# Shunpoco/mini-kube-scheduler

Measured on AMD Instinct MI355X. Metric: pod×node filter+score evals/sec and pods scheduled/sec at 100k nodes, 1/2/4/8 GPU, higher is better.
Workload: dtype u32; 1 GPU; C: 100000 nodes x 100000 pods (100000 per GPU, strong scaling), NU+NN, batched, every pair evaluated, node-sharded over 1 GPU; nodes=100000, pods=100000, pods_per_gpu=100000, plugins=NU+NN, parallelism=node-shard1

## Files before the change

mini-kube-scheduler_amd/csrc/ms_capi.cpp:

```cpp
#include <hip/hip_runtime.h>

#include <algorithm>
#include <cstdio>
#include <cstdlib>
#include <cstring>
#include <functional>
#include <mutex>
#include <new>
#include <string>
#include <type_traits>
#include <unordered_map>
#include <vector>

#include "ms_ctx.h"
#include "ms_nam_layout.h"

using namespace msgpu;

ms_ctx::~ms_ctx() {
    (void)hipSetDevice(cfg.device);
    comm_free(this);
    if (stream) (void)hipStreamSynchronize(stream);
    if (copy_stream) (void)hipStreamSynchronize(copy_stream);
}
// ... 40 lines not shown
    if (fenced) ++c->fence_seq;
    std::unordered_map<uint32_t, uint32_t> last;
    last.reserve(batch.size() * 2);
    for (uint32_t i = 0; i < batch.size(); ++i) last[batch[i].local] = i;
    std::vector<NodeDelta> uniq;
    uniq.reserve(last.size());
    for (uint32_t i = 0; i < batch.size(); ++i)
        if (last[batch[i].local] == i) uniq.push_back(batch[i]);
    int rc = ensure_delta_cap(c, (uint32_t)uniq.size());
    if (rc) return rc;
    MS_HIP(c, hipStreamSynchronize(c->stream));
    std::memcpy(c->h_deltas, uniq.data(), sizeof(NodeDelta) * uniq.size());
    MS_HIP(c, hipMemcpyAsync(c->d_deltas, c->h_deltas, sizeof(NodeDelta) * uniq.size(),
                             hipMemcpyHostToDevice, c->stream));
    MS_HIP(c, launch_apply_deltas(c->t, c->d_deltas, (uint32_t)uniq.size(), c->stream));
    MS_HIP(c, launch_build_planes(c->t, c->d_deltas, (uint32_t)uniq.size(), c->stream));
    ++c->ctx_seq;
    return MS_OK;
}

hipStream_t pick_stream(ms_ctx *c, void *s) { return s ? (hipStream_t)s : c->stream; }

int order_after_ctx_stream(ms_ctx *c, hipStream_t s) {
    const int fenced = comm_fence_reads(c, c->stream);
    if (fenced < 0) return fenced;
    if (fenced) ++c->fence_seq;
    if (s == c->stream) return MS_OK;
    if (s == c->ordered_stream && c->ordered_seq == c->ctx_seq && c->ordered_fence == c->fence_seq)
        return MS_OK;
    MS_HIP(c, made(c->ev_order.ensure()));
    hipError_t e = hipEventRecord(c->ev_order, c->stream);
// ... 246 lines not shown
        MS_HIP(c, launch_decode(d_pods + s0, nb, c->d_keys, nullptr, c->present_dev, d_res + s0, s));
        if (commit) MS_HIP(c, launch_apply_binds(c->t, d_pods + s0, nb, d_res + s0, s));
    }
    return MS_OK;
}

int sweep_locked(ms_ctx *c, uint32_t n_pods, const ms_pod_rec *d_pods, unsigned long long *keys, uint32_t *flags,
                 hipStream_t s, hipEvent_t done) {
    const uint32_t seed32 = seed32_of(c->cfg.seed);
    if (c->cfg.plugin_set == MS_PLUGINS_NU_TT_NN)
        return fail(c, MS_E_INVAL, "TaintToleration shards combine by summaries (ms_tt_summaries_device), not keys");
    if (c->cfg.plugin_set == MS_PLUGINS_NU_NN_NAM)
        return fail(c, MS_E_INVAL, "multi-term NodeAffinity shards exchange rescale tables first "
                                   "(ms_nam_segment_device, ms_nam_keys_device)");
    if (c->cfg.plugin_set == MS_PLUGINS_NU_NN) {
        MS_HIP(c, launch_sweep_pp(c->t, c->rows_dev, d_pods, n_pods, seed32, keys, nullptr, c->present_dev,
                                  c->num_cus, s, 0, done));
        return MS_OK;
    } else if (c->cfg.plugin_set == MS_PLUGINS_NU_NN_NA) {
        MS_HIP(c, launch_fill_keys(keys, n_pods, c->present_dev ? kKeyListed : 0ull, s));
        MS_HIP(c, hipMemsetAsync(flags, 0, sizeof(uint32_t) * n_pods, s));
        MS_HIP(c, launch_sweep_na(c->t, c->rows_dev, d_pods, n_pods, seed32, c->w_nn, c->w_na, keys, flags,
                                  c->num_cus, s));
    } else {
        MS_HIP(c, launch_fill_keys(keys, n_pods, c->present_dev ? kKeyListed : 0ull, s));
        if (flags) MS_HIP(c, hipMemsetAsync(flags, 0, sizeof(uint32_t) * n_pods, s));
        MS_HIP(c, launch_sweep_full(c->t, c->rows_dev, d_pods, n_pods, seed32, keys, flags, c->num_cus, s));
    }
    if (done) MS_HIP(c, hipEventRecord(done, s));
    return MS_OK;
}
// ... 10 lines not shown
    const uint32_t B = c->batch_cap;
    const bool fused = c->cfg.plugin_set == MS_PLUGINS_NU_NN;
    if (c->cfg.plugin_set == MS_PLUGINS_NU_NN_NAM) {
        int rc = nam_cycle_locked(c, n_pods, d_pods, d_res, commit, s);
        if (rc) return rc;
        if (done) MS_HIP(c, hipEventRecord(done, s));
        return MS_OK;
    }
    if (c->cfg.plugin_set == MS_PLUGINS_NU_TT_NN) {
        int rc = tt_cycle_locked(c, n_pods, d_pods, nullptr, d_res, commit, s);
        if (rc) return rc;
        if (done) MS_HIP(c, hipEventRecord(done, s));
        return MS_OK;
    }
    if (fused && c->rows_dev <= kPpMaxFusedRows) {
        MS_HIP(c, launch_sweep_pp(c->t, c->rows_dev, d_pods, n_pods, seed32_of(c->cfg.seed), nullptr, d_res,
                                  c->present_dev, c->num_cus, s, commit, done));
        return MS_OK;
    }
    const bool late_commit = commit && !plugins_stateless(c);
    for (uint32_t s0 = 0; s0 < n_pods; s0 += B) {
        const uint32_t nb = std::min(B, n_pods - s0);
        if (fused) {
            MS_HIP(c, launch_sweep_pp(c->t, c->rows_dev, d_pods + s0, nb, seed32_of(c->cfg.seed), c->d_keys,
                                      d_res + s0, c->present_dev, c->num_cus, s, commit));
            continue;
        }
        const bool want_flags = c->cfg.plugin_set != MS_PLUGINS_NU_NN;
        int rc = sweep_locked(c, nb, d_pods + s0, c->d_keys, want_flags ? c->d_flags : nullptr, s);
        if (rc) return rc;
        MS_HIP(c, decode_for(c, d_pods + s0, nb, c->d_keys, want_flags ? c->d_flags : nullptr, c->present_dev,
                             d_res + s0, s));
        if (commit && !late_commit) MS_HIP(c, launch_apply_binds(c->t, d_pods + s0, nb, d_res + s0, s));
    }
    if (late_commit) MS_HIP(c, launch_apply_binds(c->t, d_pods, n_pods, d_res, s));
    if (done) MS_HIP(c, hipEventRecord(done, s));
    return MS_OK;
}

// ... 108 lines not shown
            }
        });
    };
    ++c->ctx_seq;
    ck.count(MS_PH_CHUNKS, parts);
    for (uint32_t i = 0; i < parts; ++i) {
        ms_pod_compact *z = c->h_podz;
        par(beg(i), beg(i + 1), [&](uint32_t a, uint32_t b) {
            if constexpr (std::is_same<PodIn, ms_pod_compact>::value) {
                std::memcpy(z + a, pods + a, sizeof(ms_pod_compact) * (b - a));
            } else {
                for (uint32_t j = a; j < b; ++j) std::memcpy(&z[j], &pods[j], sizeof(ms_pod_compact));
            }
        });
        ck.lap(MS_PH_STAGE_IN);
        MS_HIP(c, launch_sweep_pp_compact(c->t, c->rows_dev, c->h_podz + beg(i), beg(i + 1) - beg(i),
                                          seed32_of(c->cfg.seed), c->h_resz + beg(i), c->present_dev, c->num_cus, s));
        MS_HIP(c, hipEventRecord(c->ev_cyc[i], s));
        ck.lap(MS_PH_LAUNCH);
        if (i > 0) {
            MS_HIP(c, hipEventSynchronize(c->ev_cyc[i - 1]));
            ck.lap(MS_PH_WAIT);
            move_out(i - 1);
            ck.lap(MS_PH_STAGE_OUT);
        }
    }
    MS_HIP(c, hipEventSynchronize(c->ev_cyc[parts - 1]));
    ck.lap(MS_PH_WAIT);
    move_out(parts - 1);
    ck.lap(MS_PH_STAGE_OUT);
    return MS_OK;
// ... 89 lines not shown
                     (void **)&t.nz_mem};
    const size_t bytes[] = {n + kColumnPad, n + kColumnPad, n + kColumnPad, n + kColumnPad, n * 4, n * 4, n * 4,
                            n * 8,          n * 8,          n * 8,          n * 8,          n * 8, n * 8};
    static_assert(sizeof(cols) / sizeof(cols[0]) == sizeof(bytes) / sizeof(bytes[0]), "one size per column");
    size_t off[sizeof(bytes) / sizeof(bytes[0])], total = 0;
    for (size_t i = 0; i < sizeof(bytes) / sizeof(bytes[0]); ++i) {
        off[i] = total;
        total += (bytes[i] + 255) & ~(size_t)255;
    }
    total = (total + (2u << 20) - 1) & ~(size_t)((2u << 20) - 1);
    bool ok = c->d_table.alloc(total);
    if (ok)
        for (size_t i = 0; i < sizeof(bytes) / sizeof(bytes[0]); ++i)
            *cols[i] = static_cast<char *>(c->d_table.get()) + off[i];
    t.gcap = (uint32_t)((n + kGroupRows - 1) / kGroupRows);
    ok = ok && c->d_planes.alloc((size_t)kPlanes * t.gcap);
    if (!ok) return bail(MS_E_OOM, "node table allocation");
    t.planes = c->d_planes;
    const size_t b = c->batch_cap;
    ok = ensure_stage(c, c->batch_cap) == MS_OK && c->d_keys.alloc(b) && c->d_flags.alloc(b) && c->d_one.alloc(1) &&
         c->d_overflow.alloc(kStatsBytes / sizeof(uint32_t));
    if (!ok) return bail(MS_E_OOM, "staging allocation");
    if (launch_init_table(t, c->stream) != hipSuccess || launch_build_planes(t, nullptr, 0, c->stream) != hipSuccess)
        return bail(MS_E_HIP, "table init launch");
    if (hipMemsetAsync(c->d_overflow, 0, kStatsBytes, c->stream) != hipSuccess) return bail(MS_E_HIP, "memset");
    if (hipStreamSynchronize(c->stream) != hipSuccess) return bail(MS_E_HIP, "table init");
    *out = c;
    return MS_OK;
}

int ms_destroy(ms_ctx *c) {
    if (!c) return MS_E_INVAL;
#ifdef MS_VSTAMPS
    {
        uint32_t st[64] = {};
        (void)hipSetDevice(c->cfg.device);
        (void)hipStreamSynchronize(c->stream);
        if (hipMemcpy(st, c->d_overflow, kStatsBytes, hipMemcpyDeviceToHost) == hipSuccess) {
// ... 680 lines not shown
```

mini-kube-scheduler_amd/csrc/ms_comm.cpp:

```cpp
#include <rccl/rccl.h>

#include <algorithm>
#include <chrono>
#include <cstdio>
#include <cstdlib>
#include <cstring>
#include <deque>
#include <new>

#include "ms_ctx.h"

#ifdef MS_COMM_LOOPBACK
#include "ms_comm_loopback.h"
#define CCL(fn) lb_##fn
#else
#define CCL(fn) fn
#endif

namespace msgpu {

namespace {

constexpr uint32_t kPipeMax = 8;
static_assert(kPipeMax <= kMaxSliceJobs, "a full drain is one slice-decode launch");
// ... 295 lines not shown
    uint32_t si = 0;
    hipStream_t X = nullptr;
    int rc = prepare_locked(c, n, s, si, X);
    if (rc) return rc;
    host_tick(m, 0, tp);
    if (co && (!m.stash.on || m.stash.X != X)) {
        rc = flush_stash(c);
        if (rc) return rc;
        m.stash = CommState::Stash{true, n, si, pods, results, X};
        return MS_OK;
    }
    ShardSlot &sl = m.slot[si];
    if (co) {
        const CommState::Stash st = m.stash;
        m.stash.on = false;
        MS_HIP(c, launch_sweep_pp2(c->t, c->rows_dev, st.pods, st.n, m.slot[st.si].keys, pods, n, sl.keys,
                                   seed32_of(c->cfg.seed), c->present_dev, c->num_cus, X, m.ev_swept[si]));
        host_tick(m, 1, tp);
        m.reads_outstanding = true;
        rc = collective_locked(c, st.si, m.ev_swept[si], st.n, st.pods, st.results, tp);
        if (rc) return rc;
        return collective_locked(c, si, nullptr, n, pods, results, tp);
    }
    const int ps = c->cfg.plugin_set;
    if (ps == MS_PLUGINS_NU_TT_NN) {
        rc = tt2_sharded_sweep(c, si, n, pods, X);
        if (rc == MS_OK && hipEventRecord(m.ev_swept[si], X) != hipSuccess) rc = fail(c, MS_E_HIP, "event record");
    } else {
        rc = sweep_locked(c, n, pods, sl.keys, ps == MS_PLUGINS_NU_NN ? nullptr : sl.flags, X, m.ev_swept[si]);
    }
    if (rc) return rc;
// ... 251 lines not shown
```

mini-kube-scheduler_amd/csrc/ms_ctx.h:

```cpp
#pragma once

#include <hip/hip_runtime.h>

#include <chrono>
#include <cstdint>
#include <memory>
#include <mutex>
#include <string>
#include <type_traits>
#include <vector>

#include "ms_copy_pool.h"
#include "ms_internal.h"
#include "ms_owned.h"

namespace msgpu {
struct CommState;

template <class T>
constexpr size_t kElemBytes = sizeof(std::conditional_t<std::is_void<T>::value, char, T>);

template <class T>
struct DevMem {
    using handle = T *;
// ... 46 lines not shown
using msgpu::DRow;
using msgpu::Event;
using msgpu::NodeDelta;
using msgpu::NodeTable;
using msgpu::PinnedBuf;
using msgpu::Stream;

struct ms_ctx {
    ms_config cfg{};
    Stream stream;
    Stream copy_stream;
    int num_cus = 0;
    NodeTable t{};
    DevBuf<void> d_table;
    DevBuf<uint32_t> d_planes;
    ~ms_ctx();

    std::unique_ptr<msgpu::CopyPool> copy_pool;

    std::mutex delta_mu;
    std::vector<NodeDelta> pending;
    std::vector<uint8_t> present;
    uint32_t present_count = 0;
    uint32_t rows_used = 0;
    uint32_t rows_dev = 0, present_dev = 0;

    std::mutex sched_mu;

    uint32_t batch_cap = 0, stage_cap = 0, compact_cap = 0;
    DevBuf<ms_pod_compact> d_podc;
// ... 117 lines not shown
```

mini-kube-scheduler_amd/csrc/ms_internal.h:

```cpp
#pragma once

#include <hip/hip_runtime.h>
#include <stdint.h>

#include "minisched_gpu.h"

namespace msgpu {

constexpr uint8_t kNodeUnschedulable = 0x01;
constexpr uint8_t kNodeAbsent = 0x80;

constexpr int kNunnThreads = 256;
constexpr int kNunnSlots = 16;
constexpr int kNunnTile = kNunnThreads * kNunnSlots;

constexpr int kFullThreads = 256;
constexpr int kFullSlots = 4;
constexpr int kFullWaveTile = 64 * kFullSlots;
constexpr int kFullTile = kFullThreads * kFullSlots;

constexpr uint32_t kGolden32 = 0x9E3779B1u;

constexpr uint32_t kColumnPad = 64;

// ... 38 lines not shown

constexpr uint32_t kGroupRows = 30;
enum : uint32_t {
    kPlaneD0 = 0,
    kPlaneD1,
    kPlaneD2,
    kPlaneD3,
    kPlaneSched,
    kPlanePresent,
    kPlaneOver,
    kPlaneDigitPres,
    kPlaneDigitSched,
    kPlanes
};

struct NodeDelta {
    uint32_t local;
    uint32_t absent;
    ms_node_rec rec;
};
static_assert(sizeof(ms_node_rec) == 64, "ms_node_rec layout");
static_assert(sizeof(ms_pod_rec) == 40, "ms_pod_rec layout");
static_assert(sizeof(ms_result) == 24, "ms_result layout");
static_assert(sizeof(ms_pod_compact) == 8, "ms_pod_compact layout");
static_assert(sizeof(ms_result_compact) == 8, "ms_result_compact layout");

constexpr unsigned long long kKeyListed = 1ull;

__host__ __device__ inline uint32_t fmix32(uint32_t h) {
    h ^= h >> 16;
// ... 36 lines not shown
};
struct NamLayout;
hipError_t launch_nam_segment(const NodeTable &t, uint32_t n_rows, const ms_pod_rec *pods, uint32_t n_pods,
                              const void *sets, uint32_t n_sets, const NamLayout &L, void *scratch, void *out,
                              hipStream_t s);
hipError_t launch_nam_identity(void *out, uint32_t n, hipStream_t s);
hipError_t launch_nam_compose(const void *in, uint32_t stride, uint32_t n, uint32_t n_pods, int32_t skip_to,
                              void *out, uint8_t *m_in, hipStream_t s);
hipError_t launch_nam_keys(const NodeTable &t, uint32_t n_rows, const ms_pod_rec *pods, uint32_t n_pods,
                           const void *sets, uint32_t n_sets, uint32_t seed32, uint32_t w_nn, uint32_t w_na,
                           const void *after, const uint8_t *m_in, uint32_t listed, const NamLayout &L,
                           void *scratch, unsigned long long *keys, hipStream_t s);

hipError_t launch_apply_deltas(const NodeTable &t, const NodeDelta *d_deltas, uint32_t n, hipStream_t s);
hipError_t launch_init_table(const NodeTable &t, hipStream_t s);
hipError_t launch_sweep_pp(const NodeTable &t, uint32_t n_rows, const ms_pod_rec *pods, uint32_t n_pods,
                           uint32_t seed32, unsigned long long *keys, ms_result *results, uint32_t present,
                           int num_cus, hipStream_t s, int commit = 0, hipEvent_t done = nullptr);
hipError_t launch_sweep_pp2(const NodeTable &t, uint32_t n_rows, const ms_pod_rec *pods1, uint32_t n1,
                            unsigned long long *keys1, const ms_pod_rec *pods2, uint32_t n2, unsigned long long *keys2,
                            uint32_t seed32, uint32_t present, int num_cus, hipStream_t s, hipEvent_t done);
hipError_t launch_sweep_pp_compact(const NodeTable &t, uint32_t n_rows, const ms_pod_compact *pods, uint32_t n_pods,
                                   uint32_t seed32, ms_result_compact *results, uint32_t present, int num_cus,
                                   hipStream_t s);
constexpr uint32_t kPpMaxFusedRows = 16u * 64u * 4u * kGroupRows;
hipError_t launch_build_planes(const NodeTable &t, const NodeDelta *d_deltas, uint32_t n, hipStream_t s);
hipError_t launch_fill_keys(unsigned long long *keys, uint32_t n, unsigned long long v, hipStream_t s);
hipError_t launch_sweep_na(const NodeTable &t, uint32_t n_rows, const ms_pod_rec *pods, uint32_t n_pods,
                           uint32_t seed32, uint32_t w_nn, uint32_t w_na, unsigned long long *keys, uint32_t *fkeys,
                           int num_cus, hipStream_t s);
hipError_t launch_decode_na(const ms_pod_rec *pods, uint32_t n_pods, const unsigned long long *keys,
                            const uint32_t *fkeys, uint32_t present_nodes, uint32_t seed32, uint32_t w_nn,
                            uint32_t w_na, ms_result *out, hipStream_t s, const uint32_t *present_dev = nullptr);
hipError_t launch_sweep_full(const NodeTable &t, uint32_t n_rows, const ms_pod_rec *pods, uint32_t n_pods,
                             uint32_t seed32, unsigned long long *keys, uint32_t *flags, int num_cus,
                             hipStream_t s);
hipError_t launch_build_drows(const NodeTable &t, uint32_t n_rows, uint32_t n_total, hipStream_t s);
hipError_t launch_decode(const ms_pod_rec *pods, uint32_t n_pods, const unsigned long long *keys,
                         const uint32_t *flags, uint32_t present_nodes, ms_result *out, hipStream_t s,
                         const uint32_t *present_dev = nullptr);

// ... 106 lines not shown
```

mini-kube-scheduler_amd/csrc/ms_sweep_pp.hip:

```cpp
#include <hip/hip_ext.h>

#include <algorithm>
#include <cstdlib>

#include "ms_device.h"

namespace msgpu {

namespace {

template <typename F>
constexpr uint32_t truth3(F f) {
    uint32_t t = 0;
    for (int i = 0; i < 8; ++i)
        if (f((i >> 2) & 1, (i >> 1) & 1, i & 1)) t |= 1u << i;
    return t;
}
constexpr uint32_t kXnorAnd = truth3([](int a, int b, int c) { return c && a == b; });
constexpr uint32_t kSelect = truth3([](int a, int b, int c) { return c ? a : b; });

constexpr uint32_t kTailShare = 4;

constexpr int kPpWords = 4;
constexpr int kPpWordsSmall = 8;
// ... 122 lines not shown
    if (__ballot(found) != 0) return (1ull << 32) | wave_max_u32_dpp(h);
    return 0;
}

__device__ __forceinline__ uint2 pod_entry(const ms_pod_rec *__restrict__ pods, uint32_t p, uint32_t seed32,
                                           uint32_t pstride, uint32_t base10) {
    const uint2 pr = *reinterpret_cast<const uint2 *>(reinterpret_cast<const char *>(pods) + (size_t)p * pstride);
    const int dig = (int)(int8_t)(pr.y & 0xFFu);
    const bool isd = (uint32_t)dig <= 9u;
    const uint32_t info = (isd ? (uint32_t)dig : 14u) | (((pr.y >> 8) & 0xFFu) ? 16u : 0u);
    const uint32_t p0 = isd ? ((uint32_t)dig + 10u - base10) % 10u : 30u;
    return make_uint2(tb_pod(seed32, pr.x), info | ((pr.y & 0xFFu) << 8) | (p0 << 16));
}

constexpr uint32_t kPpClasses = 20;
constexpr uint32_t kPpSortWords = 72;
constexpr uint32_t kPpSortMin = 80;

__device__ __forceinline__ uint32_t pod_class(uint32_t info) {
    const uint32_t p0 = (info >> 16) & 31u;
    return p0 < 10u ? p0 + ((info & 16u) ? 10u : 0u) : kPpClasses;
}

template <int KW, int NW>
__device__ __forceinline__ bool run_setup(const Word (&W)[KW], uint32_t info, uint32_t (&B)[NW * 3]) {
    const Pod qc = pod_bits(0u, info);
    uint32_t m[NW], fb = 0;
    bool has = false;
#pragma unroll
    for (int k = 0; k < NW; ++k) {
        m[k] = match10(W[k], qc);
// ... 79 lines not shown
            if (mine && u != 0u) atomicMax(&lds[pb + pi], (11ull << 32) | u);
            u64 redo = __ballot(mine && u == 0u);
            while (redo) {
                const uint32_t l = (uint32_t)__builtin_ctzll(redo);
                redo &= redo - 1ull;
                const uint32_t t = rev3(l >> 3);
                const Pod qs = pod_bits((uint32_t)__builtin_amdgcn_readlane((int)a_l, (int)(j + t)),
                                        (uint32_t)__builtin_amdgcn_readlane((int)info_l, (int)(j + t)));
                const u64 v = pod_slow<KW, NW, MODE == kModeFix>(W, Wt, TAIL && ((pb + j) >> 3) % tshare == tidx, qs);
                if (lane == 0 && v) atomicMax(&lds[pb + j + t], v);
            }
        }
    }
}

template <int KW, int NW, int MODE, bool TAIL>
__device__ __forceinline__ void sweep_range(const Word (&W)[KW], const Word &Wt, uint32_t tpt, uint32_t tshare,
                                            uint32_t tidx, const uint2 *pinfo, const uint32_t *rb, bool runs,
                                            uint32_t np, uint32_t lane, u64 *lds) {
    constexpr bool RUN = MODE != kModeGen && NW > 0 && KW == kPpWords;
    const bool cut = RUN && runs;
    for (uint32_t c = cut ? 0u : kPpClasses; c <= kPpClasses; ++c) {
        const uint32_t beg = cut ? (uint32_t)__builtin_amdgcn_readfirstlane((int)rb[c]) : 0u;
        const uint32_t end = cut ? (uint32_t)__builtin_amdgcn_readfirstlane((int)rb[c + 1]) : np;
        if (beg >= end) continue;
        uint32_t B[RUN ? NW * 3 : 1] = {};
        bool form = false;
        if constexpr (RUN)
            if (c < kPpClasses)
                form = run_setup<KW, NW>(W, (uint32_t)__builtin_amdgcn_readfirstlane((int)pinfo[beg].y), B);
        sweep_pods<KW, NW, MODE, TAIL>(W, Wt, tpt, tshare, tidx, pinfo, beg, end, form, B, lane, lds);
    }
}

__host__ __device__ inline uint32_t tail_pods(uint32_t ng, uint32_t waves) {
    if (ng == 0) return 0u;
    const uint32_t wlast = (ng + 63u) / 64u - 1u, tail_n = ng - wlast * 64u;
    const uint32_t tpt = tail_n <= 8u ? 8u : 0u;
    if (!tpt) return 0u;
    if (waves <= 4u) return tpt;
    const uint32_t wv_t = wlast % waves;
    const uint32_t tshare = kTailShare < waves - wv_t ? kTailShare : waves - wv_t;
    uint32_t L[4] = {0, 0, 0, 0};
    for (uint32_t w = 0; w < waves && w <= wlast; ++w) L[w & 3u] += 16u * ((wlast - w) / waves + 1u);
// ... 7 lines not shown
    for (uint32_t i = 0; i < tshare; ++i) L[(wv_t + i) & 3u] += eps;
    return mx() < m0 ? tpt : 0u;
}

struct PpJob2 {
    const ms_pod_rec *pods;
    u64 *keys;
    uint32_t n_pods, nblk1;
};

template <int KW, bool TP>
__global__ __launch_bounds__(64 * kPpMaxWaves) void k_sweep_nunn_pp(
    const uint32_t *__restrict__ planes, uint32_t gstride, uint32_t n_groups, uint32_t node_base,
    const ms_pod_rec *__restrict__ pods1, uint32_t n_pods1, uint32_t chunk, uint32_t seed32, u64 *__restrict__ keys1,
    int atomic_keys, ms_result *__restrict__ results, uint32_t present, NodeTable tab, int commit,
    uint32_t pstride, ms_result_compact *__restrict__ resc, PpJob2 j2, int fix_ok, uint32_t xtra) {
    extern __shared__ u64 lds[];
    uint2 *pinfo = reinterpret_cast<uint2 *>(lds + chunk + (xtra ? 8u : 0u));
    const uint32_t lane = lane_id();
    const uint32_t wv = (uint32_t)__builtin_amdgcn_readfirstlane((int)(threadIdx.x >> 6));
    const bool second = j2.pods && blockIdx.x >= j2.nblk1;
    const ms_pod_rec *__restrict__ pods = second ? j2.pods : pods1;
    const uint32_t n_pods = second ? j2.n_pods : n_pods1;
    u64 *__restrict__ keys = second ? j2.keys : keys1;
    const uint32_t bi = second ? blockIdx.x - j2.nblk1 : blockIdx.x;
    const uint32_t pbeg = bi * chunk + min(bi, xtra) * 8u;
    const uint32_t pend = min(n_pods, pbeg + chunk + (bi < xtra ? 8u : 0u));
    const uint32_t np = pend > pbeg ? pend - pbeg : 0u;
    uint32_t *cnt = reinterpret_cast<uint32_t *>(pinfo + chunk + (xtra ? 8u : 0u));
    uint32_t *rb = cnt + 24, *sb = cnt + 48;
    const bool runs = KW == kPpWords && chunk >= kPpSortMin;
    if (!runs) {
        for (uint32_t i = threadIdx.x; i < np; i += blockDim.x) {
            lds[i] = 0;
            uint2 e = pod_entry(pods, pbeg + i, seed32, pstride, node_base % 10u);
            e.y |= i << 21;
            pinfo[i] = e;
        }
    } else {
        if (threadIdx.x < 24u) cnt[threadIdx.x] = 0u;
        __syncthreads();
        for (uint32_t i = threadIdx.x; i < np; i += blockDim.x) {
            uint2 e = pod_entry(pods, pbeg + i, seed32, pstride, node_base % 10u);
            e.y |= atomicAdd(&cnt[pod_class(e.y)], 1u) << 21;
            reinterpret_cast<uint2 *>(lds)[i] = e;
        }
        __syncthreads();
        if (threadIdx.x <= kPpClasses) {
            uint32_t a = 0, b = 0, na = 0, nb = 0;
            for (uint32_t c = 0; c < kPpClasses; ++c) {
                const uint32_t n = cnt[c], full = n & ~7u;
                if (c == threadIdx.x) a = na, b = nb;
                na += full;
                nb += n - full;
            }
            if (threadIdx.x == kPpClasses) {
                a = na, b = nb;
                rb[kPpClasses + 1] = np;
            }
            rb[threadIdx.x] = a;
            sb[threadIdx.x] = na + b;
        }
        __syncthreads();
        for (uint32_t i = threadIdx.x; i < np; i += blockDim.x) {
            const uint2 e = reinterpret_cast<const uint2 *>(lds)[i];
            const uint32_t c = pod_class(e.y), rank = e.y >> 21;
// ... 45 lines not shown
        Wt.d3 = in ? planes[kPlaneD3 * gstride + g] : 0u;
        Wt.sched = in ? planes[kPlaneSched * gstride + g] : 0u;
        Wt.pres = in ? planes[kPlanePresent * gstride + g] : 0u;
        Wt.hb = (node_base + g * kGroupRows) * kG24;
        Wt.dsched = Wt.dpres = 0u;
        over = over || (in && (planes[kPlaneOver * gstride + g] & 1u) != 0u);
    }
    const bool gen = __ballot(over) != 0;
    const int mode = gen ? kModeGen : (fix_ok && __ballot(misaligned) == 0) ? kModeFix : kModeFast;
    __syncthreads();
    if (np && (nw || tpt)) {
        switch (nw * 6 + mode * 2 + (tpt ? 1 : 0)) {
#define MS_PP_CASE1(N, M, T)                                                                                     \
    case 6 * N + 2 * M + T:                                                                                      \
        if constexpr (N <= KW && (N > 0 || T))                                                                   \
            sweep_range<KW, (N <= KW ? N : KW), M, T>(W, Wt, tpt, tshare, wv - wv_t, pinfo, rb, runs, np, lane, lds); \
        break;
#define MS_PP_CASE(N)        \
    MS_PP_CASE1(N, 0, false) \
    MS_PP_CASE1(N, 0, true)  \
    MS_PP_CASE1(N, 1, false) \
    MS_PP_CASE1(N, 1, true)  \
    MS_PP_CASE1(N, 2, false) \
    MS_PP_CASE1(N, 2, true)
            MS_PP_CASE(0)
            MS_PP_CASE(1)
            MS_PP_CASE(2)
            MS_PP_CASE(3)
            MS_PP_CASE(4)
            MS_PP_CASE(5)
            MS_PP_CASE(6)
            MS_PP_CASE(7)
            MS_PP_CASE(8)
#undef MS_PP_CASE
#undef MS_PP_CASE1
            default:
                break;
        }
    }
    __syncthreads();
    for (uint32_t i = threadIdx.x; i < np; i += blockDim.x) {
        const u64 v = lds[i];
        const uint2 pe = pinfo[i];
        const uint32_t po = pbeg + (pe.y >> 21);
        u64 key = present ? kKeyListed : 0ull;
        if (v) {
            const uint32_t h = (uint32_t)v;
            key = make_key((uint32_t)(v >> 32) - 1u, h, tb_unhash(pe.x, h));
        }
        if (keys) {
            if (!atomic_keys) keys[po] = key;
            else if (key) atomicMax(&keys[po], key);
        }
        if (results || resc) {
// ... 8 lines not shown
                rc.plugin_mask = (uint8_t)r.plugin_mask;
                resc[po] = rc;
            }
            if (commit && r.code == MS_CODE_SUCCESS) {
                if (resc) {
                    const ms_pod_rec z = {};
                    add_pod(tab, (uint32_t)r.node - tab.base, z, +1);
                } else {
                    add_pod(tab, (uint32_t)r.node - tab.base, pods[po], +1);
                }
            }
        }
    }
}

__device__ __forceinline__ void build_group(const NodeTable &t, uint32_t g) {
    uint32_t d[4] = {0, 0, 0, 0}, sched = 0, pres = 0, isdig = 0, misal = 0;
    for (uint32_t s = 0; s < kGroupRows; ++s) {
        const uint32_t r = g * kGroupRows + s;
        if (r >= t.cap) break;
        const uint32_t f = t.flags[r], dg = t.digit[r];
        const uint32_t v = dg <= 9u ? dg : 15u;
#pragma unroll
        for (int b = 0; b < 4; ++b) d[b] |= ((v >> b) & 1u) << s;
        if (!(f & kNodeAbsent)) {
            pres |= 1u << s;
            if (!(f & kNodeUnschedulable)) sched |= 1u << s;
            if (v <= 9u) {
                isdig |= 1u << s;
                if (v != (t.base + r) % 10u) misal = 2u;
// ... 14 lines not shown
    t.planes[kPlaneD0 * st + g] = d[0];
    t.planes[kPlaneD1 * st + g] = d[1];
    t.planes[kPlaneD2 * st + g] = d[2];
    t.planes[kPlaneD3 * st + g] = d[3];
    t.planes[kPlaneSched * st + g] = sched;
    t.planes[kPlanePresent * st + g] = pres;
}

__global__ void k_build_planes(NodeTable t, const NodeDelta *__restrict__ deltas, uint32_t n) {
    const uint32_t i = blockIdx.x * blockDim.x + threadIdx.x;
    if (i >= n) return;
    const uint32_t g = deltas ? deltas[i].local / kGroupRows : i;
    if (g < t.gcap) build_group(t, g);
}

inline uint32_t cdiv(uint32_t a, uint32_t b) { return (a + b - 1) / b; }

}

hipError_t launch_build_planes(const NodeTable &t, const NodeDelta *d_deltas, uint32_t n, hipStream_t s) {
    if (!t.planes) return hipSuccess;
    if (!d_deltas) n = t.gcap;
    if (n == 0) return hipSuccess;
    hipLaunchKernelGGL(k_build_planes, dim3(cdiv(n, 256)), dim3(256), 0, s, t, d_deltas, n);
    return hipGetLastError();
}

constexpr uint32_t kPpMaxChunk = 2048;

namespace {
hipError_t sweep_pp_impl(const NodeTable &t, uint32_t n_rows, const ms_pod_rec *pods, uint32_t n_pods,
                         uint32_t seed32, unsigned long long *keys, ms_result *results, uint32_t present, int num_cus,
                         hipStream_t s, int commit, hipEvent_t done, uint32_t pstride, ms_result_compact *resc,
                         const ms_pod_rec *pods2 = nullptr, uint32_t n_pods2 = 0, unsigned long long *keys2 = nullptr) {
    if (n_pods == 0 && n_pods2 == 0) return done ? hipEventRecord(done, s) : hipSuccess;
    const uint32_t n_all = n_pods + (pods2 ? n_pods2 : 0u);
    if (!t.planes) return hipErrorInvalidValue;
    const uint32_t n_groups = cdiv(n_rows, kGroupRows);
    const char *wenv = getenv("MINISCHED_PP_WORDS");
    const uint32_t cus_ = (uint32_t)(num_cus > 0 ? num_cus : 256);
    bool small = n_groups <= kPpSmallGroups && n_all >= 1024u * cus_ && !getenv("MINISCHED_PP_WAVES");
    if (wenv) small = n_groups <= kPpSmallGroups && atoi(wenv) == 8;
    const uint32_t KW = small ? (uint32_t)kPpWordsSmall : (uint32_t)kPpWords;
    const uint32_t waves_needed = std::max(1u, cdiv(n_groups, 64u * KW));
    uint32_t W = 1;
    if (waves_needed == 2) W = 2;
// ... 22 lines not shown
                nblk1 = slots;
            }
        }
    }
    const dim3 grid(nblk1 + (pods2 ? (xtra ? nblk1 : cdiv(n_pods2, chunk)) : 0u), gy);
    constexpr int fix_ok = 1;
    const PpJob2 j2 = {pods2, reinterpret_cast<u64 *>(keys2), n_pods2, nblk1};
    if (pods2 && (gy > 1 || results || resc || !keys || !keys2)) return hipErrorInvalidValue;
    if (gy > 1) {
        if (!keys || resc) return hipErrorInvalidValue;
        hipError_t e = hipMemsetAsync(keys, 0, sizeof(unsigned long long) * n_pods, s);
        if (e != hipSuccess) return e;
        hipLaunchKernelGGL((k_sweep_nunn_pp<kPpWords, false>), grid, dim3(64 * W),
                           chunk * (sizeof(u64) + sizeof(uint2)) + kPpSortWords * sizeof(uint32_t), s, t.planes,
                           t.gcap, n_groups, t.base, pods, n_pods, chunk, seed32, keys, 1, (ms_result *)nullptr, present,
                           t, 0, (uint32_t)sizeof(ms_pod_rec), (ms_result_compact *)nullptr, PpJob2{}, fix_ok, 0u);
        e = hipGetLastError();
        if (e == hipSuccess && results) e = launch_decode(pods, n_pods, keys, nullptr, present, results, s);
        if (e == hipSuccess && results && commit) e = launch_apply_binds(t, pods, n_pods, results, s);
        if (e == hipSuccess && done) e = hipEventRecord(done, s);
        return e;
    }
    const uint32_t lds = (chunk + (xtra ? 8u : 0u)) * (sizeof(u64) + sizeof(uint2)) + kPpSortWords * sizeof(uint32_t);
    unsigned long long *kk = (results || resc) ? nullptr : keys;
    const int cm = (results || resc) ? commit : 0;
    const bool tp = KW == (uint32_t)kPpWords && tail_pods(n_groups, W) != 0u;
#define MS_PP_LAUNCH(KWV, TPV)                                                                                     \
    hipExtLaunchKernelGGL((k_sweep_nunn_pp<KWV, TPV>), grid, dim3(64 * W), lds, s, nullptr, done, 0, t.planes, t.gcap, \
                          n_groups, t.base, pods, n_pods, chunk, seed32, kk, 0, results, present, t, cm, pstride, resc, j2, \
                          fix_ok, xtra)
    if (KW == (uint32_t)kPpWordsSmall) {
        MS_PP_LAUNCH(kPpWordsSmall, false);
    } else {
        if (tp) MS_PP_LAUNCH(kPpWords, true);
        else MS_PP_LAUNCH(kPpWords, false);
    }
#undef MS_PP_LAUNCH
    return hipGetLastError();
}
}

hipError_t launch_sweep_pp(const NodeTable &t, uint32_t n_rows, const ms_pod_rec *pods, uint32_t n_pods,
                           uint32_t seed32, unsigned long long *keys, ms_result *results, uint32_t present,
                           int num_cus, hipStream_t s, int commit, hipEvent_t done) {
    return sweep_pp_impl(t, n_rows, pods, n_pods, seed32, keys, results, present, num_cus, s, commit, done,
                         (uint32_t)sizeof(ms_pod_rec), nullptr);
}

hipError_t launch_sweep_pp2(const NodeTable &t, uint32_t n_rows, const ms_pod_rec *pods1, uint32_t n1,
                            unsigned long long *keys1, const ms_pod_rec *pods2, uint32_t n2, unsigned long long *keys2,
                            uint32_t seed32, uint32_t present, int num_cus, hipStream_t s, hipEvent_t done) {
    if (n_rows > kPpMaxFusedRows) return hipErrorInvalidValue;
    return sweep_pp_impl(t, n_rows, pods1, n1, seed32, keys1, nullptr, present, num_cus, s, 0, done,
                         (uint32_t)sizeof(ms_pod_rec), nullptr, pods2, n2, keys2);
}

hipError_t launch_sweep_pp_compact(const NodeTable &t, uint32_t n_rows, const ms_pod_compact *pods, uint32_t n_pods,
                                   uint32_t seed32, ms_result_compact *results, uint32_t present, int num_cus,
                                   hipStream_t s) {
    static_assert(sizeof(ms_pod_compact) == 8 && sizeof(ms_result_compact) == 8, "compact records");
    if (n_rows > kPpMaxFusedRows || !results) return hipErrorInvalidValue;
    return sweep_pp_impl(t, n_rows, reinterpret_cast<const ms_pod_rec *>(pods), n_pods, seed32, nullptr, nullptr,
                         present, num_cus, s, 1, nullptr, (uint32_t)sizeof(ms_pod_compact), results);
}

}
```

Measured before the change: 50340 billion pod×node evals/s.

## Precompute per-class candidate node lists and sweep pods against compacted lists

Adds a k_build_cand kernel that, after each plane rebuild, compacts node entries matching each of the 20 pod classes into padded per-class tiled lists with offsets in a header. The pod-parallel sweep then evaluates pods of classes with non-empty lists only against their candidate nodes, instead of scanning all node groups with bitmask planes. This targets wasted work on non-matching nodes. In exchange it adds an extra kernel launch on every delta update, extra device memory, and more LDS use for the header.

```diff
diff --git a/mini-kube-scheduler_amd/csrc/ms_capi.cpp b/mini-kube-scheduler_amd/csrc/ms_capi.cpp
--- a/mini-kube-scheduler_amd/csrc/ms_capi.cpp
+++ b/mini-kube-scheduler_amd/csrc/ms_capi.cpp
@@ -78,7 +78,7 @@
     MS_HIP(c, hipMemcpyAsync(c->d_deltas, c->h_deltas, sizeof(NodeDelta) * uniq.size(),
                              hipMemcpyHostToDevice, c->stream));
     MS_HIP(c, launch_apply_deltas(c->t, c->d_deltas, (uint32_t)uniq.size(), c->stream));
-    MS_HIP(c, launch_build_planes(c->t, c->d_deltas, (uint32_t)uniq.size(), c->stream));
+    MS_HIP(c, launch_build_planes(c->t, c->d_cand, c->d_deltas, (uint32_t)uniq.size(), c->stream));
     ++c->ctx_seq;
     return MS_OK;
 }
@@ -355,7 +355,7 @@
         return fail(c, MS_E_INVAL, "multi-term NodeAffinity shards exchange rescale tables first "
                                    "(ms_nam_segment_device, ms_nam_keys_device)");
     if (c->cfg.plugin_set == MS_PLUGINS_NU_NN) {
-        MS_HIP(c, launch_sweep_pp(c->t, c->rows_dev, d_pods, n_pods, seed32, keys, nullptr, c->present_dev,
+        MS_HIP(c, launch_sweep_pp(c->t, c->d_cand, c->rows_dev, d_pods, n_pods, seed32, keys, nullptr, c->present_dev,
                                   c->num_cus, s, 0, done));
         return MS_OK;
     } else if (c->cfg.plugin_set == MS_PLUGINS_NU_NN_NA) {
@@ -396,7 +396,7 @@
         return MS_OK;
     }
     if (fused && c->rows_dev <= kPpMaxFusedRows) {
-        MS_HIP(c, launch_sweep_pp(c->t, c->rows_dev, d_pods, n_pods, seed32_of(c->cfg.seed), nullptr, d_res,
+        MS_HIP(c, launch_sweep_pp(c->t, c->d_cand, c->rows_dev, d_pods, n_pods, seed32_of(c->cfg.seed), nullptr, d_res,
                                   c->present_dev, c->num_cus, s, commit, done));
         return MS_OK;
     }
@@ -404,7 +404,7 @@
     for (uint32_t s0 = 0; s0 < n_pods; s0 += B) {
         const uint32_t nb = std::min(B, n_pods - s0);
         if (fused) {
-            MS_HIP(c, launch_sweep_pp(c->t, c->rows_dev, d_pods + s0, nb, seed32_of(c->cfg.seed), c->d_keys,
+            MS_HIP(c, launch_sweep_pp(c->t, c->d_cand, c->rows_dev, d_pods + s0, nb, seed32_of(c->cfg.seed), c->d_keys,
                                       d_res + s0, c->present_dev, c->num_cus, s, commit));
             continue;
         }
@@ -543,7 +543,7 @@
             }
         });
         ck.lap(MS_PH_STAGE_IN);
-        MS_HIP(c, launch_sweep_pp_compact(c->t, c->rows_dev, c->h_podz + beg(i), beg(i + 1) - beg(i),
+        MS_HIP(c, launch_sweep_pp_compact(c->t, c->d_cand, c->rows_dev, c->h_podz + beg(i), beg(i + 1) - beg(i),
                                           seed32_of(c->cfg.seed), c->h_resz + beg(i), c->present_dev, c->num_cus, s));
         MS_HIP(c, hipEventRecord(c->ev_cyc[i], s));
         ck.lap(MS_PH_LAUNCH);
@@ -663,14 +663,14 @@
         for (size_t i = 0; i < sizeof(bytes) / sizeof(bytes[0]); ++i)
             *cols[i] = static_cast<char *>(c->d_table.get()) + off[i];
     t.gcap = (uint32_t)((n + kGroupRows - 1) / kGroupRows);
-    ok = ok && c->d_planes.alloc((size_t)kPlanes * t.gcap);
+    ok = ok && c->d_planes.alloc((size_t)kPlanes * t.gcap) && c->d_cand.alloc(cand_words(t.cap));
     if (!ok) return bail(MS_E_OOM, "node table allocation");
     t.planes = c->d_planes;
     const size_t b = c->batch_cap;
     ok = ensure_stage(c, c->batch_cap) == MS_OK && c->d_keys.alloc(b) && c->d_flags.alloc(b) && c->d_one.alloc(1) &&
          c->d_overflow.alloc(kStatsBytes / sizeof(uint32_t));
     if (!ok) return bail(MS_E_OOM, "staging allocation");
-    if (launch_init_table(t, c->stream) != hipSuccess || launch_build_planes(t, nullptr, 0, c->stream) != hipSuccess)
+    if (launch_init_table(t, c->stream) != hipSuccess || launch_build_planes(t, c->d_cand, nullptr, 0, c->stream) != hipSuccess)
         return bail(MS_E_HIP, "table init launch");
     if (hipMemsetAsync(c->d_overflow, 0, kStatsBytes, c->stream) != hipSuccess) return bail(MS_E_HIP, "memset");
     if (hipStreamSynchronize(c->stream) != hipSuccess) return bail(MS_E_HIP, "table init");
diff --git a/mini-kube-scheduler_amd/csrc/ms_comm.cpp b/mini-kube-scheduler_amd/csrc/ms_comm.cpp
--- a/mini-kube-scheduler_amd/csrc/ms_comm.cpp
+++ b/mini-kube-scheduler_amd/csrc/ms_comm.cpp
@@ -333,7 +333,7 @@
     if (co) {
         const CommState::Stash st = m.stash;
         m.stash.on = false;
-        MS_HIP(c, launch_sweep_pp2(c->t, c->rows_dev, st.pods, st.n, m.slot[st.si].keys, pods, n, sl.keys,
+        MS_HIP(c, launch_sweep_pp2(c->t, c->d_cand, c->rows_dev, st.pods, st.n, m.slot[st.si].keys, pods, n, sl.keys,
                                    seed32_of(c->cfg.seed), c->present_dev, c->num_cus, X, m.ev_swept[si]));
         host_tick(m, 1, tp);
         m.reads_outstanding = true;
diff --git a/mini-kube-scheduler_amd/csrc/ms_ctx.h b/mini-kube-scheduler_amd/csrc/ms_ctx.h
--- a/mini-kube-scheduler_amd/csrc/ms_ctx.h
+++ b/mini-kube-scheduler_amd/csrc/ms_ctx.h
@@ -84,6 +84,7 @@
     NodeTable t{};
     DevBuf<void> d_table;
     DevBuf<uint32_t> d_planes;
+    DevBuf<uint32_t> d_cand;
     ~ms_ctx();
 
     std::unique_ptr<msgpu::CopyPool> copy_pool;
diff --git a/mini-kube-scheduler_amd/csrc/ms_internal.h b/mini-kube-scheduler_amd/csrc/ms_internal.h
--- a/mini-kube-scheduler_amd/csrc/ms_internal.h
+++ b/mini-kube-scheduler_amd/csrc/ms_internal.h
@@ -76,6 +76,13 @@
     kPlanes
 };
 
+constexpr uint32_t kCandClasses = 20;
+constexpr uint32_t kCandTile = 192;
+constexpr uint32_t kCandHeader = 64;
+__host__ __device__ inline size_t cand_words(uint32_t cap) {
+    return (size_t)kCandHeader + 2u * (size_t)cap + kCandClasses * kCandTile;
+}
+
 struct NodeDelta {
     uint32_t local;
     uint32_t absent;
@@ -142,17 +149,18 @@
 
 hipError_t launch_apply_deltas(const NodeTable &t, const NodeDelta *d_deltas, uint32_t n, hipStream_t s);
 hipError_t launch_init_table(const NodeTable &t, hipStream_t s);
-hipError_t launch_sweep_pp(const NodeTable &t, uint32_t n_rows, const ms_pod_rec *pods, uint32_t n_pods,
+hipError_t launch_sweep_pp(const NodeTable &t, const uint32_t *cand, uint32_t n_rows, const ms_pod_rec *pods, uint32_t n_pods,
                            uint32_t seed32, unsigned long long *keys, ms_result *results, uint32_t present,
                            int num_cus, hipStream_t s, int commit = 0, hipEvent_t done = nullptr);
-hipError_t launch_sweep_pp2(const NodeTable &t, uint32_t n_rows, const ms_pod_rec *pods1, uint32_t n1,
+hipError_t launch_sweep_pp2(const NodeTable &t, const uint32_t *cand, uint32_t n_rows, const ms_pod_rec *pods1, uint32_t n1,
                             unsigned long long *keys1, const ms_pod_rec *pods2, uint32_t n2, unsigned long long *keys2,
                             uint32_t seed32, uint32_t present, int num_cus, hipStream_t s, hipEvent_t done);
-hipError_t launch_sweep_pp_compact(const NodeTable &t, uint32_t n_rows, const ms_pod_compact *pods, uint32_t n_pods,
+hipError_t launch_sweep_pp_compact(const NodeTable &t, const uint32_t *cand, uint32_t n_rows, const ms_pod_compact *pods, uint32_t n_pods,
                                    uint32_t seed32, ms_result_compact *results, uint32_t present, int num_cus,
                                    hipStream_t s);
 constexpr uint32_t kPpMaxFusedRows = 16u * 64u * 4u * kGroupRows;
-hipError_t launch_build_planes(const NodeTable &t, const NodeDelta *d_deltas, uint32_t n, hipStream_t s);
+hipError_t launch_build_planes(const NodeTable &t, uint32_t *cand, const NodeDelta *d_deltas, uint32_t n,
+                               hipStream_t s);
 hipError_t launch_fill_keys(unsigned long long *keys, uint32_t n, unsigned long long v, hipStream_t s);
 hipError_t launch_sweep_na(const NodeTable &t, uint32_t n_rows, const ms_pod_rec *pods, uint32_t n_pods,
                            uint32_t seed32, uint32_t w_nn, uint32_t w_na, unsigned long long *keys, uint32_t *fkeys,
diff --git a/mini-kube-scheduler_amd/csrc/ms_sweep_pp.hip b/mini-kube-scheduler_amd/csrc/ms_sweep_pp.hip
--- a/mini-kube-scheduler_amd/csrc/ms_sweep_pp.hip
+++ b/mini-kube-scheduler_amd/csrc/ms_sweep_pp.hip
@@ -160,7 +160,7 @@
 }
 
 constexpr uint32_t kPpClasses = 20;
-constexpr uint32_t kPpSortWords = 72;
+constexpr uint32_t kPpSortWords = 96;
 constexpr uint32_t kPpSortMin = 80;
 
 __device__ __forceinline__ uint32_t pod_class(uint32_t info) {
@@ -270,20 +270,92 @@
     }
 }
 
+__device__ __forceinline__ uint32_t list_tiles(const uint32_t *hdr, uint32_t info, uint32_t *off) {
+    const uint32_t y = (uint32_t)__builtin_amdgcn_readfirstlane((int)info);
+    const uint32_t lc = (y & 15u) + ((y & 16u) ? kCandClasses / 2u : 0u);
+    const uint32_t o = (uint32_t)__builtin_amdgcn_readfirstlane((int)hdr[lc]);
+    if (off) *off = o;
+    return ((uint32_t)__builtin_amdgcn_readfirstlane((int)hdr[lc + 1]) - o) / kCandTile;
+}
+
+template <int NT>
+__device__ __forceinline__ void sweep_list_pods(const uint32_t (&B)[3 * kPpWords], const uint2 *pinfo, uint32_t beg,
+                                                uint32_t end, uint32_t lane, u64 *lds) {
+    for (uint32_t pb = beg; pb < end; pb += 64) {
+        const uint32_t nblk = min(64u, end - pb);
+        const uint32_t a_l = lane < nblk ? pinfo[pb + lane].x : 0u;
+        for (uint32_t j = 0; j < nblk; j += 8) {
+            uint32_t r[8];
+            if (nblk - j >= 8u) {
+#pragma unroll
+                for (int t = 0; t < 8; ++t) {
+                    const uint32_t A = (uint32_t)__builtin_amdgcn_readlane((int)a_l, (int)(j + t));
+                    uint32_t h = 0;
+#pragma unroll
+                    for (int i = 0; i < 3 * NT; ++i) h = max(h, mix32(B[i] + A));
+                    r[t] = h;
+                }
+            } else {
+#pragma unroll
+                for (int t = 0; t < 8; ++t) {
+                    r[t] = 0;
+                    if (j + (uint32_t)t < nblk) {
+                        const uint32_t A = (uint32_t)__builtin_amdgcn_readlane((int)a_l, (int)(j + t));
+#pragma unroll
+                        for (int i = 0; i < 3 * NT; ++i) r[t] = max(r[t], mix32(B[i] + A));
+                    }
+                }
+            }
+            const uint32_t u = reduce8(r, lane);
+            const uint32_t pi = j + rev3(lane >> 3);
+            if ((lane & 7u) == 0u && pi < nblk) atomicMax(&lds[pb + pi], (11ull << 32) | u);
+        }
+    }
+}
+
+__device__ __forceinline__ void sweep_lists(const uint32_t *__restrict__ cand, const uint32_t *hdr,
+                                            const uint2 *pinfo, const uint32_t *rb, uint32_t wv, uint32_t waves,
+                                            uint32_t lane, u64 *lds) {
+    for (uint32_t c = 0; c < kPpClasses; ++c) {
+        const uint32_t beg = (uint32_t)__builtin_amdgcn_readfirstlane((int)rb[c]);
+        const uint32_t end = (uint32_t)__builtin_amdgcn_readfirstlane((int)rb[c + 1]);
+        if (beg >= end) continue;
+        uint32_t off;
+        const uint32_t ntile = list_tiles(hdr, pinfo[beg].y, &off);
+        for (uint32_t t0 = wv; t0 < ntile; t0 += kPpWords * waves) {
+            const uint32_t nt = min((uint32_t)kPpWords, (ntile - t0 + waves - 1u) / waves);
+            uint32_t B[3 * kPpWords];
+#pragma unroll
+            for (int k = 0; k < kPpWords; ++k) {
+                const uint32_t *e = cand + kCandHeader + off + (t0 + k * waves) * kCandTile + lane;
+#pragma unroll
+                for (int i = 0; i < 3; ++i) B[3 * k + i] = (uint32_t)k < nt ? e[i * 64] : 0u;
+            }
+            switch (nt) {
+                case 1: sweep_list_pods<1>(B, pinfo, beg, end, lane, lds); break;
+                case 2: sweep_list_pods<2>(B, pinfo, beg, end, lane, lds); break;
+                case 3: sweep_list_pods<3>(B, pinfo, beg, end, lane, lds); break;
+                default: sweep_list_pods<4>(B, pinfo, beg, end, lane, lds); break;
+            }
+        }
+    }
+}
+
 template <int KW, int NW, int MODE, bool TAIL>
 __device__ __forceinline__ void sweep_range(const Word (&W)[KW], const Word &Wt, uint32_t tpt, uint32_t tshare,
                                             uint32_t tidx, const uint2 *pinfo, const uint32_t *rb, bool runs,
-                                            uint32_t np, uint32_t lane, u64 *lds) {
+                                            bool lists, const uint32_t *hdr, uint32_t np, uint32_t lane, u64 *lds) {
     constexpr bool RUN = MODE != kModeGen && NW > 0 && KW == kPpWords;
-    const bool cut = RUN && runs;
+    const bool cut = lists || (RUN && runs);
     for (uint32_t c = cut ? 0u : kPpClasses; c <= kPpClasses; ++c) {
         const uint32_t beg = cut ? (uint32_t)__builtin_amdgcn_readfirstlane((int)rb[c]) : 0u;
         const uint32_t end = cut ? (uint32_t)__builtin_amdgcn_readfirstlane((int)rb[c + 1]) : np;
         if (beg >= end) continue;
+        if (lists && c < kPpClasses && list_tiles(hdr, pinfo[beg].y, nullptr) != 0u) continue;
         uint32_t B[RUN ? NW * 3 : 1] = {};
         bool form = false;
         if constexpr (RUN)
-            if (c < kPpClasses)
+            if (!lists && c < kPpClasses)
                 form = run_setup<KW, NW>(W, (uint32_t)__builtin_amdgcn_readfirstlane((int)pinfo[beg].y), B);
         sweep_pods<KW, NW, MODE, TAIL>(W, Wt, tpt, tshare, tidx, pinfo, beg, end, form, B, lane, lds);
     }
@@ -321,7 +393,8 @@
     const uint32_t *__restrict__ planes, uint32_t gstride, uint32_t n_groups, uint32_t node_base,
     const ms_pod_rec *__restrict__ pods1, uint32_t n_pods1, uint32_t chunk, uint32_t seed32, u64 *__restrict__ keys1,
     int atomic_keys, ms_result *__restrict__ results, uint32_t present, NodeTable tab, int commit,
-    uint32_t pstride, ms_result_compact *__restrict__ resc, PpJob2 j2, int fix_ok, uint32_t xtra) {
+    uint32_t pstride, ms_result_compact *__restrict__ resc, PpJob2 j2, int fix_ok, uint32_t xtra,
+    const uint32_t *__restrict__ cand) {
     extern __shared__ u64 lds[];
     uint2 *pinfo = reinterpret_cast<uint2 *>(lds + chunk + (xtra ? 8u : 0u));
     const uint32_t lane = lane_id();
@@ -335,8 +408,9 @@
     const uint32_t pend = min(n_pods, pbeg + chunk + (bi < xtra ? 8u : 0u));
     const uint32_t np = pend > pbeg ? pend - pbeg : 0u;
     uint32_t *cnt = reinterpret_cast<uint32_t *>(pinfo + chunk + (xtra ? 8u : 0u));
-    uint32_t *rb = cnt + 24, *sb = cnt + 48;
+    uint32_t *rb = cnt + 24, *sb = cnt + 48, *hdr = cnt + 72;
     const bool runs = KW == kPpWords && chunk >= kPpSortMin;
+    const bool lists = runs && cand != nullptr && gridDim.y == 1u;
     if (!runs) {
         for (uint32_t i = threadIdx.x; i < np; i += blockDim.x) {
             lds[i] = 0;
@@ -346,6 +420,8 @@
         }
     } else {
         if (threadIdx.x < 24u) cnt[threadIdx.x] = 0u;
+        if (lists)
+            for (uint32_t i = threadIdx.x; i <= kCandClasses; i += blockDim.x) hdr[i] = cand[i];
         __syncthreads();
         for (uint32_t i = threadIdx.x; i < np; i += blockDim.x) {
             uint2 e = pod_entry(pods, pbeg + i, seed32, pstride, node_base % 10u);
@@ -356,7 +432,7 @@
         if (threadIdx.x <= kPpClasses) {
             uint32_t a = 0, b = 0, na = 0, nb = 0;
             for (uint32_t c = 0; c < kPpClasses; ++c) {
-                const uint32_t n = cnt[c], full = n & ~7u;
+                const uint32_t n = cnt[c], full = lists ? n : n & ~7u;
                 if (c == threadIdx.x) a = na, b = nb;
                 na += full;
                 nb += n - full;
@@ -432,7 +508,8 @@
 #define MS_PP_CASE1(N, M, T)                                                                                     \
     case 6 * N + 2 * M + T:                                                                                      \
         if constexpr (N <= KW && (N > 0 || T))                                                                   \
-            sweep_range<KW, (N <= KW ? N : KW), M, T>(W, Wt, tpt, tshare, wv - wv_t, pinfo, rb, runs, np, lane, lds); \
+            sweep_range<KW, (N <= KW ? N : KW), M, T>(W, Wt, tpt, tshare, wv - wv_t, pinfo, rb, runs, lists, hdr, np, \
+                                                      lane, lds);                                               \
         break;
 #define MS_PP_CASE(N)        \
     MS_PP_CASE1(N, 0, false) \
@@ -456,6 +533,8 @@
                 break;
         }
     }
+    if constexpr (KW == kPpWords)
+        if (np && lists) sweep_lists(cand, hdr, pinfo, rb, wv, waves, lane, lds);
     __syncthreads();
     for (uint32_t i = threadIdx.x; i < np; i += blockDim.x) {
         const u64 v = lds[i];
@@ -494,6 +573,8 @@
     }
 }
 
+__host__ __device__ inline uint32_t cdiv(uint32_t a, uint32_t b) { return (a + b - 1) / b; }
+
 __device__ __forceinline__ void build_group(const NodeTable &t, uint32_t g) {
     uint32_t d[4] = {0, 0, 0, 0}, sched = 0, pres = 0, isdig = 0, misal = 0;
     for (uint32_t s = 0; s < kGroupRows; ++s) {
@@ -538,22 +619,92 @@
     if (g < t.gcap) build_group(t, g);
 }
 
-inline uint32_t cdiv(uint32_t a, uint32_t b) { return (a + b - 1) / b; }
-
-}
-
-hipError_t launch_build_planes(const NodeTable &t, const NodeDelta *d_deltas, uint32_t n, hipStream_t s) {
+__device__ __forceinline__ uint32_t cand_mask(const NodeTable &t, uint32_t g, uint32_t c) {
+    const uint32_t st = t.gcap, v = c % 10u;
+    const uint32_t d0 = t.planes[kPlaneD0 * st + g], d1 = t.planes[kPlaneD1 * st + g];
+    const uint32_t d2 = t.planes[kPlaneD2 * st + g], d3 = t.planes[kPlaneD3 * st + g];
+    const uint32_t f = t.planes[(c >= 10u ? kPlanePresent : kPlaneSched) * st + g];
+    return f & ((v & 1u) ? d0 : ~d0) & ((v & 2u) ? d1 : ~d1) & ((v & 4u) ? d2 : ~d2) & ((v & 8u) ? d3 : ~d3);
+}
+
+constexpr uint32_t kCandThreads = 1024;
+
+__global__ __launch_bounds__(kCandThreads) void k_build_cand(NodeTable t, uint32_t *__restrict__ cand) {
+    __shared__ uint32_t cnt[kCandClasses], wsum[kCandThreads / 64], first;
+    const uint32_t c = blockIdx.x, tid = threadIdx.x, lane = tid & 63u, wv = tid >> 6;
+    if (tid < kCandClasses) cnt[tid] = 0u;
+    __syncthreads();
+    uint32_t n[kCandClasses] = {};
+    for (uint32_t g = tid; g < t.gcap; g += kCandThreads) {
+#pragma unroll
+        for (uint32_t k = 0; k < kCandClasses; ++k) n[k] += (uint32_t)__popc(cand_mask(t, g, k));
+    }
+#pragma unroll
+    for (uint32_t k = 0; k < kCandClasses; ++k) {
+        const uint32_t sum = wave_sum_u32_dpp(n[k]);
+        if (lane == 0u && sum) atomicAdd(&cnt[k], sum);
+    }
+    __syncthreads();
+    uint32_t off = 0;
+    for (uint32_t k = 0; k < c; ++k) off += cdiv(cnt[k], kCandTile) * kCandTile;
+    const uint32_t len = cnt[c], padded = cdiv(len, kCandTile) * kCandTile;
+    if (tid == 0u) {
+        cand[c] = off;
+        cand[kCandClasses + 1u + c] = len;
+        if (c + 1u == kCandClasses) cand[kCandClasses] = off + padded;
+    }
+    uint32_t *ent = cand + kCandHeader + off;
+    uint32_t done = 0;
+    for (uint32_t g0 = 0; g0 < t.gcap; g0 += kCandThreads) {
+        const uint32_t g = g0 + tid;
+        uint32_t m = g < t.gcap ? cand_mask(t, g, c) : 0u;
+        const uint32_t k = (uint32_t)__popc(m);
+        uint32_t incl = k;
+#pragma unroll
+        for (uint32_t d = 1; d < 64u; d <<= 1) {
+            const uint32_t up = (uint32_t)__shfl_up((int)incl, d, 64);
+            if (lane >= d) incl += up;
+        }
+        if (lane == 63u) wsum[wv] = incl;
+        __syncthreads();
+        uint32_t before = 0, total = 0;
+        for (uint32_t w = 0; w < kCandThreads / 64; ++w) {
+            if (w < wv) before += wsum[w];
+            total += wsum[w];
+        }
+        uint32_t pos = done + before + incl - k;
+        while (m) {
+            const uint32_t slot = (uint32_t)__builtin_ctz(m);
+            m &= m - 1u;
+            const uint32_t e = (t.base + g * kGroupRows + slot) * kG24;
+            if (pos == 0u) first = e;
+            if (pos < len) ent[pos] = e;
+            ++pos;
+        }
+        done += total;
+        __syncthreads();
+    }
+    for (uint32_t i = len + tid; i < padded; i += kCandThreads) ent[i] = first;
+}
+
+}
+
+hipError_t launch_build_planes(const NodeTable &t, uint32_t *cand, const NodeDelta *d_deltas, uint32_t n,
+                               hipStream_t s) {
     if (!t.planes) return hipSuccess;
     if (!d_deltas) n = t.gcap;
     if (n == 0) return hipSuccess;
     hipLaunchKernelGGL(k_build_planes, dim3(cdiv(n, 256)), dim3(256), 0, s, t, d_deltas, n);
+    hipError_t e = hipGetLastError();
+    if (e != hipSuccess || !cand) return e;
+    hipLaunchKernelGGL(k_build_cand, dim3(kCandClasses), dim3(kCandThreads), 0, s, t, cand);
     return hipGetLastError();
 }
 
 constexpr uint32_t kPpMaxChunk = 2048;
 
 namespace {
-hipError_t sweep_pp_impl(const NodeTable &t, uint32_t n_rows, const ms_pod_rec *pods, uint32_t n_pods,
+hipError_t sweep_pp_impl(const NodeTable &t, const uint32_t *cand, uint32_t n_rows, const ms_pod_rec *pods, uint32_t n_pods,
                          uint32_t seed32, unsigned long long *keys, ms_result *results, uint32_t present, int num_cus,
                          hipStream_t s, int commit, hipEvent_t done, uint32_t pstride, ms_result_compact *resc,
                          const ms_pod_rec *pods2 = nullptr, uint32_t n_pods2 = 0, unsigned long long *keys2 = nullptr) {
@@ -606,7 +757,8 @@
         hipLaunchKernelGGL((k_sweep_nunn_pp<kPpWords, false>), grid, dim3(64 * W),
                            chunk * (sizeof(u64) + sizeof(uint2)) + kPpSortWords * sizeof(uint32_t), s, t.planes,
                            t.gcap, n_groups, t.base, pods, n_pods, chunk, seed32, keys, 1, (ms_result *)nullptr, present,
-                           t, 0, (uint32_t)sizeof(ms_pod_rec), (ms_result_compact *)nullptr, PpJob2{}, fix_ok, 0u);
+                           t, 0, (uint32_t)sizeof(ms_pod_rec), (ms_result_compact *)nullptr, PpJob2{}, fix_ok, 0u,
+                           (const uint32_t *)nullptr);
         e = hipGetLastError();
         if (e == hipSuccess && results) e = launch_decode(pods, n_pods, keys, nullptr, present, results, s);
         if (e == hipSuccess && results && commit) e = launch_apply_binds(t, pods, n_pods, results, s);
@@ -620,7 +772,7 @@
 #define MS_PP_LAUNCH(KWV, TPV)                                                                                     \
     hipExtLaunchKernelGGL((k_sweep_nunn_pp<KWV, TPV>), grid, dim3(64 * W), lds, s, nullptr, done, 0, t.planes, t.gcap, \
                           n_groups, t.base, pods, n_pods, chunk, seed32, kk, 0, results, present, t, cm, pstride, resc, j2, \
-                          fix_ok, xtra)
+                          fix_ok, xtra, cand)
     if (KW == (uint32_t)kPpWordsSmall) {
         MS_PP_LAUNCH(kPpWordsSmall, false);
     } else {
@@ -632,27 +784,27 @@
 }
 }
 
-hipError_t launch_sweep_pp(const NodeTable &t, uint32_t n_rows, const ms_pod_rec *pods, uint32_t n_pods,
+hipError_t launch_sweep_pp(const NodeTable &t, const uint32_t *cand, uint32_t n_rows, const ms_pod_rec *pods, uint32_t n_pods,
                            uint32_t seed32, unsigned long long *keys, ms_result *results, uint32_t present,
                            int num_cus, hipStream_t s, int commit, hipEvent_t done) {
-    return sweep_pp_impl(t, n_rows, pods, n_pods, seed32, keys, results, present, num_cus, s, commit, done,
+    return sweep_pp_impl(t, cand, n_rows, pods, n_pods, seed32, keys, results, present, num_cus, s, commit, done,
                          (uint32_t)sizeof(ms_pod_rec), nullptr);
 }
 
-hipError_t launch_sweep_pp2(const NodeTable &t, uint32_t n_rows, const ms_pod_rec *pods1, uint32_t n1,
+hipError_t launch_sweep_pp2(const NodeTable &t, const uint32_t *cand, uint32_t n_rows, const ms_pod_rec *pods1, uint32_t n1,
                             unsigned long long *keys1, const ms_pod_rec *pods2, uint32_t n2, unsigned long long *keys2,
                             uint32_t seed32, uint32_t present, int num_cus, hipStream_t s, hipEvent_t done) {
     if (n_rows > kPpMaxFusedRows) return hipErrorInvalidValue;
-    return sweep_pp_impl(t, n_rows, pods1, n1, seed32, keys1, nullptr, present, num_cus, s, 0, done,
+    return sweep_pp_impl(t, cand, n_rows, pods1, n1, seed32, keys1, nullptr, present, num_cus, s, 0, done,
                          (uint32_t)sizeof(ms_pod_rec), nullptr, pods2, n2, keys2);
 }
 
-hipError_t launch_sweep_pp_compact(const NodeTable &t, uint32_t n_rows, const ms_pod_compact *pods, uint32_t n_pods,
+hipError_t launch_sweep_pp_compact(const NodeTable &t, const uint32_t *cand, uint32_t n_rows, const ms_pod_compact *pods, uint32_t n_pods,
                                    uint32_t seed32, ms_result_compact *results, uint32_t present, int num_cus,
                                    hipStream_t s) {
     static_assert(sizeof(ms_pod_compact) == 8 && sizeof(ms_result_compact) == 8, "compact records");
     if (n_rows > kPpMaxFusedRows || !results) return hipErrorInvalidValue;
-    return sweep_pp_impl(t, n_rows, reinterpret_cast<const ms_pod_rec *>(pods), n_pods, seed32, nullptr, nullptr,
+    return sweep_pp_impl(t, cand, n_rows, reinterpret_cast<const ms_pod_rec *>(pods), n_pods, seed32, nullptr, nullptr,
                          present, num_cus, s, 1, nullptr, (uint32_t)sizeof(ms_pod_compact), results);
 }
 
```

Result: faster. 54000 billion pod×node evals/s, median of 6 (+7.3%).
